# mlcolab/Pathfinder.jl

Hardware: AMD Instinct MI355X
Metric: ELBO draws/sec (multipathfinder hot path: fit + ELBO + pool + PSIS + resample) (higher is better)
Workload: dtype f64

## Files before the change

### pathfinder.jl_amd/csrc/elbo_qf_kernel.hip

```cpp
#include <type_traits>
#include <stdio.h>
#include <stdlib.h>
#include "pfmi_common.h"
#include "elbo_args.h"
#ifndef QF_PROF
#define QF_PROF 0
#endif

#ifndef QF_WAVES
#define QF_WAVES 8
#endif
#define QF_THREADS (QF_WAVES * 64)
#ifndef QF_NG
#define QF_NG 2
#endif
#ifndef QF_ABLATE
#define QF_ABLATE 0
#endif
#ifndef QF_NG2_MAXKC
#define QF_NG2_MAXKC 20
#endif
#ifndef QF_PRIO_FAIR
#define QF_PRIO_FAIR 8
#endif
#ifndef QF_PRIO_YOUNG
#define QF_PRIO_YOUNG 0
#endif
#ifndef QF_SETPRIO
#define QF_SETPRIO 0
#endif
#define QF_MIN_FRONT 1024
static_assert(QF_MIN_FRONT >= 2 * PF_ICDF_BFE_FRONT, "the look-up's front guard");
template <int KC> struct qf_chb { static constexpr int v = (KC > 20) ? 8 : 16; };

#pragma clang fp contract(off)

typedef double qf_d4 __attribute__((ext_vector_type(4)));
__device__ __forceinline__ qf_d4 qf_mfma16(double a, double b, qf_d4 c) { return __builtin_amdgcn_mfma_f64_16x16x4f64(a, b, c, 0, 0, 0); }
__device__ __forceinline__ double qf_mfma4(double a, double b, double c) { return __builtin_amdgcn_mfma_f64_4x4x4f64(a, b, c, 0, 0, 0); }

__host__ __device__ constexpr int qf_nconst(int KC, int RPAD) { return 4 + KC + KC * KC + RPAD + RPAD * KC + KC; }

template <int TGT>
__device__ __forceinline__ void qf_row_ac(const ElboArgs &A, const double *mu, int i, double &a, double &c) {
    if (TGT == 1) { a = A.t_a[i]; c = mu[i] - A.t_mean[i]; }
    else if (TGT == 2) { a = (i >= 1) ? 1.0 : 0.0; c = mu[i]; }
    else { a = 0.0; c = 0.0; }
}

template <int KC>
__device__ __forceinline__ int qf_vh_pos(int lrow, int col) {
    const int bl = lrow >> 4, rr = lrow & 15, q = rr >> 2, r = rr & 3, T = col >> 2, i = col & 3;
    return (((bl * 4 + r) * (KC / 4) + T) << 4) + q * 4 + i;
}

struct QfKernArgs { ElboArgs A; int ch_blocks, nchunks, groups_per_wg, ngroups, n_whole, n_tail, ndep; double *cshare; unsigned *cflag; unsigned epoch; };
#ifndef QF_SHARE_SPINS
#define QF_SHARE_SPINS 2000000
#endif
template <int KC, int TGT, int RPAD, int NG>
__global__ __launch_bounds__(QF_THREADS) void pf_elbo_qf_kernel(ElboArgs A, int ch_blocks, int nchunks, int groups_per_wg, int ngroups, int n_whole,
                                                                  int n_tail, int ndep, double *, unsigned *, unsigned) {
    extern __shared__ __attribute__((aligned(16))) double lds[];
#if QF_PROF
    const long long qf_t0 = wall_clock64();
    long long qf_tb = 0, qf_te = 0, qf_tp = 0, qf_last = 0;
#endif
    constexpr int NT = KC / 4, TR = RPAD / 4, NC = qf_nconst(KC, RPAD);
    constexpr int QF_CHB = qf_chb<KC>::v;
    constexpr bool FOLD = !(NG == 2 && KC >= 16);
    constexpr int PRE = (QF_CHB * 16 * KC + QF_THREADS - 1) / QF_THREADS;
    const int tid = threadIdx.x, wv = tid >> 6, lane = tid & 63, q = lane >> 4, c = lane & 15, l3 = lane & 3;
    const int d = A.d, nblk = (d + 15) >> 4;
    int slot = blockIdx.y, role = 0;
    int g_begin = blockIdx.x * groups_per_wg, g_cap = groups_per_wg;
    if (n_tail > 0 && slot >= n_whole) {
        constexpr int SL = QF_WAVES * NG, NPG_ = (TGT != 0) ? (KC + 1 + 15) / 16 : 0;
        int tail_f;
        if (slot < n_whole + n_tail) { role = 1; tail_f = slot - n_whole; g_begin = 0; g_cap = SL - NPG_; }
        else {
            const int t = slot - n_whole - n_tail;
            role = 2; tail_f = t / ndep;
            g_begin = (SL - NPG_) + (t - tail_f * ndep) * SL; g_cap = SL;
        }
        slot = n_whole + tail_f;
    }
    const int p = A.points[slot];
    const size_t blkidx = A.by_point ? (size_t)p : (size_t)slot;
    double *out_lp = A.logp + blkidx * A.log_stride, *out_lq = A.logq + blkidx * A.log_stride;
    constexpr int NPG = (TGT != 0) ? (KC + 1 + 15) / 16 : 0;
    const int npg = (role == 2) ? 0 : NPG;
    const int g_end = (g_begin + g_cap < ngroups) ? g_begin + g_cap : ngroups;
    const int nlb = (npg + (g_end - g_begin) + QF_WAVES * NG - 1) / (QF_WAVES * NG);
    if (A.status[p] != PFMI_FIT_OK) {
        for (int64_t n = (int64_t)g_begin * 16 + tid; n < (int64_t)g_end * 16 && n < A.N; n += QF_THREADS) {
            out_lp[n] = NAN; out_lq[n] = NAN;
        }
        return;
    }
    const int vh_sz = ch_blocks * 16 * KC, rs_sz = ch_blocks * 48;
    const int buf_stride = (nchunks > 1) ? vh_sz + rs_sz : 0;
    const int stage_sz = (nchunks > 1 ? 2 : 1) * (vh_sz + rs_sz);
    const int fix_off = stage_sz > QF_MIN_FRONT ? stage_sz : QF_MIN_FRONT;
    double *t_s = lds + fix_off;
    double *cn_s = t_s + KC * KC;
    double *g_s = cn_s + NC;
    double2 *icdf = reinterpret_cast<double2 *>(g_s + RPAD * RPAD + ((KC * KC + NC + RPAD * RPAD) & 1));

    const double *Vh = A.vh + (size_t)p * d * KC, *mu = A.mu + (size_t)p * d, *sqa = A.sqrt_alpha + (size_t)p * d;
    auto stage_direct = [&](int ck, int buf) {
        const int row0 = ck * ch_blocks * 16;
        double *vs = lds + buf * buf_stride, *rs = vs + vh_sz;
        const int npair = ch_blocks * 8 * KC;
        const int lim = (d - row0) * KC;
        const double2 *src = reinterpret_cast<const double2 *>(Vh + (size_t)row0 * KC);
        constexpr int U = 6;
        for (int j0 = tid; j0 < npair; j0 += QF_THREADS * U) {
            double2 v[U];
#pragma unroll
            for (int u = 0; u < U; ++u) {
                const int j = j0 + u * QF_THREADS, jc = (2 * j + 1 < lim) ? j : (lim >> 1) - 1;
                v[u] = src[jc];
            }
#pragma unroll
            for (int u = 0; u < U; ++u) {
                const int j = j0 + u * QF_THREADS, idx = 2 * j;
                if (j < npair) {
                    const int lrow = idx / KC, col = idx - lrow * KC;
                    const double2 val = (idx < lim) ? v[u] : make_double2(0.0, 0.0);
                    *reinterpret_cast<double2 *>(vs + qf_vh_pos<KC>(lrow, col)) = val;
                }
            }
        }
        for (int l0 = tid; l0 < ch_blocks * 16; l0 += QF_THREADS * 2) {
            double a[2], cc[2], s[2];
#pragma unroll
            for (int u = 0; u < 2; ++u) {
                const int lrow = l0 + u * QF_THREADS, row = row0 + lrow, rc = row < d ? row : d - 1;
                qf_row_ac<TGT>(A, mu, rc, a[u], cc[u]);
                s[u] = sqa[rc];
            }
#pragma unroll
            for (int u = 0; u < 2; ++u) {
                const int lrow = l0 + u * QF_THREADS, row = row0 + lrow;
                if (lrow < ch_blocks * 16) {
                    const bool in = row < d;
                    double *o = rs + (lrow >> 4) * 48 + (lrow & 15);
                    o[0] = in ? a[u] * s[u] * s[u] : 0.0; o[16] = in ? 2.0 * a[u] * cc[u] * s[u] : 0.0; o[32] = in ? s[u] : 0.0;
                }
            }
        }
    };
    {
        const double *T = A.tmat + (size_t)p * KC * KC;
        for (int i = tid; i < KC * KC; i += QF_THREADS) t_s[i] = T[i];
        for (int i = tid; i < NC; i += QF_THREADS) cn_s[i] = 0.0;
        if (RPAD > 0) for (int i = tid; i < RPAD * RPAD; i += QF_THREADS) g_s[i] = A.t_g[i];
        pf_icdf_load(icdf);
        stage_direct(0, 0);
    }
    const int rho = 4 * (c & 3) + (c >> 2);
    constexpr bool HREG = !(NG == 2 && KC >= 16);
    const double *Vc = A.vchol + (size_t)p * KC * KC;
    auto head_op = [&](const int which, const int r) -> double {
        const int b = 4 * q + r;
        if (which == 0) { double v = (rho == b) ? 1.0 : 0.0; if (rho < KC && b < KC) v = Vc[b * KC + rho]; return v; }
        const int i1 = 16 + rho, b1 = 16 + b;
        if (which == 1) return (i1 < KC) ? Vc[b * KC + i1] : 0.0;
        double v1 = (i1 == b1) ? 1.0 : 0.0;
        if (i1 < KC && b1 < KC) v1 = Vc[b1 * KC + i1];
        return v1;
    };
    double a_h00[HREG ? 4 : 1], a_h10[HREG ? 4 : 1], a_h11[HREG ? 4 : 1];
    if (HREG) {
#pragma unroll
        for (int r = 0; r < 4; ++r) {
            a_h00[HREG ? r : 0] = head_op(0, r);
            a_h10[HREG ? r : 0] = (KC > 16) ? head_op(1, r) : 0.0;
            a_h11[HREG ? r : 0] = (KC > 16) ? head_op(2, r) : 0.0;
        }
    }
    auto hop = [&](const int which, const int r) -> double {
        if (HREG) return which == 0 ? a_h00[HREG ? r : 0] : (which == 1 ? a_h10[HREG ? r : 0] : a_h11[HREG ? r : 0]);
        return head_op(which, r);
    };
    const uint64_t seed = A.seeds[slot];
    const uint32_t k0 = (uint32_t)seed, k1 = (uint32_t)(seed >> 32);
    const double logdet = A.logdet[p];
    __syncthreads();
#if QF_PROF
    qf_tp = wall_clock64() - qf_t0; qf_last = wall_clock64();
#endif
#if QF_PRIO_YOUNG
    if (wv >= 4) __builtin_amdgcn_s_setprio(1);
#endif
    if (TGT == 2) {
        if (tid == 0) { cn_s[1] = mu[0]; cn_s[2] = sqa[0]; }
        if (tid < KC) cn_s[4 + KC + KC * KC + RPAD + RPAD * KC + tid] = Vh[tid];
    }

    int cur = 0;
    for (int lb = 0; lb < nlb; ++lb) {
        bool pseudo[NG], active[NG];
        int sl[NG];
        int64_t nl[NG];
        uint32_t n[NG];
        double accw[NG][NT], acc3[NG][NT], acc4[NG][TR > 0 ? TR : 1];
        double usq[NG], q12[NG], z00[NG], u0[NG][4];
        bool any_active = false, any_pseudo = false, any_real = false;
#pragma unroll
        for (int g = 0; g < NG; ++g) {
            sl[g] = (lb * QF_WAVES + wv) * NG + g;
            pseudo[g] = sl[g] < npg;
            const int grp = g_begin + sl[g] - npg;
            active[g] = pseudo[g] || grp < g_end;
            nl[g] = (int64_t)grp * 16 + c;
            n[g] = (uint32_t)(A.n0 + nl[g]);
            any_active |= active[g]; any_pseudo |= pseudo[g]; any_real |= active[g] && !pseudo[g];
#pragma unroll
            for (int T = 0; T < NT; ++T) { accw[g][T] = 0.0; acc3[g][T] = 0.0; }
#pragma unroll
            for (int T = 0; T < (TR > 0 ? TR : 1); ++T) acc4[g][T] = 0.0;
            usq[g] = 0.0; q12[g] = 0.0; z00[g] = 0.0;
#pragma unroll
            for (int r = 0; r < 4; ++r) u0[g][r] = 0.0;
        }
        struct Pend { uint32_t x[4]; double dp[4]; double2 c01[4], c23[4]; };
        const uint32_t icdf_adj = pf_icdf_adj_bfe<PF_ICDF_NB_LDS>(icdf);
        auto gen_issue = [&](const int g, const int blk, Pend &P) {
#if QF_ABLATE == 1
#pragma unroll
            for (int r = 0; r < 4; ++r) { P.x[r] = 0x40000000u | (n[g] + blk); P.dp[r] = 1e-3 * (blk + r); P.c01[r] = make_double2(0.1, 0.2); P.c23[r] = make_double2(0.3, 0.4); }
#elif QF_ABLATE == 2
            pf_philox_normals(n[g], (uint32_t)(blk * 4 + q), 0u, 0u, k0, k1, P.x);
#pragma unroll
            for (int r = 0; r < 4; ++r) { P.dp[r] = (double)P.x[r] * 0x1p-32; P.c01[r] = make_double2(0.1, 0.2); P.c23[r] = make_double2(0.3, 0.4); }
#else
            pf_philox_normals(n[g], (uint32_t)(blk * 4 + q), 0u, 0u, k0, k1, P.x);
#pragma unroll
            for (int r = 0; r < 4; ++r) pf_icdf_issue_bfe<PF_ICDF_NB_LDS>(P.x[r], icdf_adj, P.dp[r], P.c01[r], P.c23[r]);
#endif
        };
        for (int ck = 0; ck < nchunks; ++ck) {
            double pre[PRE], pr_s = 0.0, pr_a = 0.0, pr_c = 0.0;
            const int nck = (ck + 1 < nchunks) ? ck + 1 : 0;
            const bool do_pre = (nchunks > 1) && (ck + 1 < nchunks || lb + 1 < nlb);
            if (do_pre) {
                const int row0 = nck * QF_CHB * 16;
                int tid_p = tid;
                asm volatile("" : "+v"(tid_p));
#pragma unroll
                for (int e = 0; e < PRE; ++e) {
                    const int idx = tid_p + e * QF_THREADS;
                    const int lrow = idx / KC, row = row0 + lrow;
                    pre[e] = (idx < QF_CHB * 16 * KC && row < d) ? Vh[(size_t)row0 * KC + idx] : 0.0;
                }
                if (tid_p < QF_CHB * 16) {
                    const int row = row0 + tid_p;
                    if (row < d) { qf_row_ac<TGT>(A, mu, row, pr_a, pr_c); pr_s = sqa[row]; }
                }
            }
            if (any_active) {
                const double *vs = lds + cur * buf_stride, *rs = vs + vh_sz;
                const int blk0 = ck * ch_blocks;
                const int nb = (nblk - blk0 < ch_blocks) ? nblk - blk0 : ch_blocks;
                struct Ops { double av[4][NT]; double wd[4][TR > 0 ? TR : 1]; double rs[12]; };
                auto load_ops = [&](const int bl, Ops &o) {
                    const double *rp = rs + bl * 48 + 4 * q;
                    const double *ap = vs + ((bl * 4) * NT << 4) + q * 4 + l3;
#pragma unroll
                    for (int r = 0; r < 4; ++r) {
#pragma unroll
                        for (int T = 0; T < NT; ++T) o.av[r][T] = ap[(r * NT + T) << 4];
                        o.rs[r] = rp[r]; o.rs[4 + r] = rp[16 + r]; o.rs[8 + r] = rp[32 + r];
                    }
                    if (TGT == 1 && RPAD > 0) {
                        const double *wp = A.t_wd16 + ((size_t)(blk0 + bl) * 16 + 4 * q) * 16 + l3;
#pragma unroll
                        for (int r = 0; r < 4; ++r)
#pragma unroll
                            for (int T = 0; T < TR; ++T) o.wd[r][T] = wp[r * 16 + 4 * T];
                    }
                };
                auto contract = [&](const int g, const double (&z)[4], const Ops &o, const bool with_w) {
#if QF_SETPRIO
                    __builtin_amdgcn_s_setprio(QF_SETPRIO);
#endif
                    double bp[4], bs[4];
#pragma unroll
                    for (int r = 0; r < 4; ++r) {
                        bp[r] = 0.0; bs[r] = 0.0;
                        if (TGT != 0) bp[r] = (with_w && FOLD) ? fma(o.rs[r], z[r], o.rs[4 + r]) : o.rs[r] * z[r];
                        if (TGT == 1 && RPAD > 0) bs[r] = o.rs[8 + r] * z[r];
                    }
                    __builtin_amdgcn_sched_barrier(0);
#pragma unroll
                    for (int r = 0; r < 4; ++r) {
                        if (TGT != 0) q12[g] = fma((with_w && FOLD) ? bp[r] : bp[r] + o.rs[4 + r], z[r], q12[g]);
#pragma unroll
                        for (int T = 0; T < NT; ++T) {
                            if (with_w) accw[g][T] = qf_mfma4(o.av[r][T], z[r], accw[g][T]);
                            if (TGT != 0) acc3[g][T] = qf_mfma4(o.av[r][T], bp[r], acc3[g][T]);
                        }
                        if (TGT == 1 && RPAD > 0) {
#pragma unroll
                            for (int T = 0; T < TR; ++T) acc4[g][T] = qf_mfma4(o.wd[r][T], bs[r], acc4[g][T]);
                        }
                    }
#if QF_SETPRIO
                    __builtin_amdgcn_s_setprio(0);
#endif
                };
                auto normals = [&](const int g, const int blk, double (&z)[4]) {
                    uint32_t x[4];
                    pf_philox_normals(n[g], (uint32_t)(blk * 4 + q), 0u, 0u, k0, k1, x);
                    pf_icdf4(x, n[g], (uint32_t)(blk * 4 + q), 0u, k0, k1, icdf, z);
                    if (blk == nblk - 1) {
#pragma unroll
                        for (int r = 0; r < 4; ++r) z[r] = (blk * 16 + 4 * q + r < d) ? z[r] : 0.0;
                    }
#pragma unroll
                    for (int r = 0; r < 4; ++r) usq[g] = fma(z[r], z[r], usq[g]);
                    if (blk == 0) {
                        qf_d4 h = {0.0, 0.0, 0.0, 0.0};
#pragma unroll
                        for (int r = 0; r < 4; ++r) { u0[g][r] = z[r]; h = qf_mfma16(hop(0, r), z[r], h); }
#pragma unroll
                        for (int r = 0; r < 4; ++r) z[r] = h[r];
                        z00[g] = z[0];
                    } else if (KC > 16 && blk == 1) {
                        qf_d4 h = {0.0, 0.0, 0.0, 0.0};
#pragma unroll
                        for (int r = 0; r < 4; ++r) h = qf_mfma16(hop(1, r), u0[g][r], h);
#pragma unroll
                        for (int r = 0; r < 4; ++r) h = qf_mfma16(hop(2, r), z[r], h);
#pragma unroll
                        for (int r = 0; r < 4; ++r) z[r] = h[r];
                    }
                };
                auto finish = [&](const int g, const int blk, const Pend &P, double (&z)[4], auto special_tag) {
                    constexpr bool SPECIAL = decltype(special_tag)::value;
#pragma unroll
                    for (int r = 0; r < 4; ++r) z[r] = pf_icdf_finish(P.x[r], P.dp[r], P.c01[r], P.c23[r]);
                    if (__builtin_expect(__any(pf_icdf_miss4(P.x)), 0))
                        pf_icdf4_fix(P.x, n[g], (uint32_t)(blk * 4 + q), 0u, k0, k1, z);
                    if (SPECIAL) {
                        if (blk == nblk - 1) {
#pragma unroll
                            for (int r = 0; r < 4; ++r) z[r] = (blk * 16 + 4 * q + r < d) ? z[r] : 0.0;
                        }
#pragma unroll
                        for (int r = 0; r < 4; ++r) usq[g] = fma(z[r], z[r], usq[g]);
                        if (blk == 0) {
                            qf_d4 h = {0.0, 0.0, 0.0, 0.0};
#pragma unroll
                            for (int r = 0; r < 4; ++r) { u0[g][r] = z[r]; h = qf_mfma16(hop(0, r), z[r], h); }
#pragma unroll
                            for (int r = 0; r < 4; ++r) z[r] = h[r];
                            z00[g] = z[0];
                        } else if (KC > 16 && blk == 1) {
                            qf_d4 h = {0.0, 0.0, 0.0, 0.0};
#pragma unroll
                            for (int r = 0; r < 4; ++r) h = qf_mfma16(hop(1, r), u0[g][r], h);
#pragma unroll
                            for (int r = 0; r < 4; ++r) h = qf_mfma16(hop(2, r), z[r], h);
#pragma unroll
                            for (int r = 0; r < 4; ++r) z[r] = h[r];
                        }
                    } else {
#pragma unroll
                        for (int r = 0; r < 4; ++r) usq[g] = fma(z[r], z[r], usq[g]);
                    }
                };
                auto pseudo_cols = [&](const int g, const int blk, const int bl, double (&z)[4]) {
                    const int j = 16 * sl[g] + c;
#pragma unroll
                    for (int r = 0; r < 4; ++r) {
                        const int row = blk * 16 + 4 * q + r;
                        double v = 0.0;
                        if (j < KC) v = vs[qf_vh_pos<KC>(bl * 16 + 4 * q + r, j)];
                        else if (j == KC && row < d) {
                            double aa, cc;
                            qf_row_ac<TGT>(A, mu, row, aa, cc);
                            v = cc / sqa[row];
                        }
                        z[r] = v;
                    }
                };
                if (any_pseudo) {
                    for (int bl = 0; bl < nb; ++bl) {
                        Ops oa;
                        load_ops(bl, oa);
#pragma unroll
                        for (int g = 0; g < NG; ++g) {
                            if (!active[g]) continue;
                            double z[4];
                            if (pseudo[g]) { pseudo_cols(g, blk0 + bl, bl, z); contract(g, z, oa, false); }
                            else { normals(g, blk0 + bl, z); contract(g, z, oa, true); }
                        }
                    }
                } else {
                    auto block_body_seq = [&](const int bl, auto special_tag) {
                        const int blk = blk0 + bl;
                        double z[NG][4];
#pragma unroll
                        for (int g = 0; g < NG; ++g) {
                            Pend pp;
                            gen_issue(g, blk, pp);
                            finish(g, blk, pp, z[g], special_tag);
                        }
                        const double *rp = rs + bl * 48 + 4 * q;
                        const double *ap = vs + ((bl * 4) * NT << 4) + q * 4 + l3;
#pragma unroll
                        for (int r = 0; r < 4; ++r) {
                            double av[NT];
#pragma unroll
                            for (int T = 0; T < NT; ++T) av[T] = ap[(r * NT + T) << 4];
                            const double r0 = rp[r], r1 = rp[16 + r];
#pragma unroll
                            for (int g = 0; g < NG; ++g) {
                                const double zr = z[g][r];
                                double bp = 0.0;
                                if (TGT != 0) {
                                    bp = r0 * zr;
                                    q12[g] = fma(bp + r1, zr, q12[g]);
                                }
#pragma unroll
                                for (int T = 0; T < NT; ++T) {
                                    accw[g][T] = qf_mfma4(av[T], zr, accw[g][T]);
                                    if (TGT != 0) acc3[g][T] = qf_mfma4(av[T], bp, acc3[g][T]);
                                }
                            }
                            if (TGT == 1 && RPAD > 0) {
                                const double *wp = A.t_wd16 + ((size_t)(blk0 + bl) * 16 + 4 * q + r) * 16 + l3;
                                double wd[TR > 0 ? TR : 1];
#pragma unroll
                                for (int T = 0; T < TR; ++T) wd[T] = wp[4 * T];
                                const double r2 = rp[32 + r];
#pragma unroll
                                for (int g = 0; g < NG; ++g) {
                                    const double bs = r2 * z[g][r];
#pragma unroll
                                    for (int T = 0; T < TR; ++T) acc4[g][T] = qf_mfma4(wd[T], bs, acc4[g][T]);
                                }
                            }
                        }
                    };
                    auto block_body = [&](const int bl, auto special_tag) {
                        if constexpr (NG == 2 && KC >= 16) { block_body_seq(bl, special_tag); return; }
                        const int blk = blk0 + bl;
                        Ops oa;
                        load_ops(bl, oa);
                        __builtin_amdgcn_sched_barrier(0);
                        Pend pp[NG];
                        double z[NG][4];
#pragma unroll
                        for (int g = 0; g < NG; ++g) gen_issue(g, blk, pp[g]);
#pragma unroll
                        for (int g = 0; g < NG; ++g) {
                            finish(g, blk, pp[g], z[g], special_tag);
#if QF_ABLATE == 3
                            q12[g] += z[g][0] + z[g][1] + z[g][2] + z[g][3] + oa.av[0][0] + oa.rs[0];
#else
                            contract(g, z[g], oa, true);
#endif
                        }
                    };
                    __builtin_amdgcn_s_waitcnt(0xC07F);
                    auto prio_turn = [&](const int blk) {
#if QF_PRIO_FAIR
                        if ((blk & (QF_PRIO_FAIR - 1)) == 0) {
                            if (((blk / QF_PRIO_FAIR) ^ (wv >> 2) ^ lb) & 1) __builtin_amdgcn_s_setprio(1); else __builtin_amdgcn_s_setprio(0);
                        }
#endif
                    };
                    if constexpr (NG == 2 && KC >= 16) {
                        for (int bl = 0; bl < nb; ++bl) {
                            const int blk = blk0 + bl;
                            prio_turn(blk);
                            if (__builtin_expect((blk == 0) | (blk == nblk - 1) | (KC > 16 && blk == 1), 0)) block_body(bl, std::true_type{});
                            else block_body(bl, std::false_type{});
                        }
                    } else {
                        constexpr int LEAD = (KC > 16) ? 2 : 1;
                        const int s_lo = (LEAD - blk0 <= 0) ? 0 : (LEAD - blk0 < nb ? LEAD - blk0 : nb);
                        const int s_hi = (blk0 + nb == nblk) ? (nb - 1 > s_lo ? nb - 1 : s_lo) : nb;
#pragma unroll
                        for (int bl = 0; bl < LEAD; ++bl)
                            if (bl < s_lo) { prio_turn(blk0 + bl); block_body(bl, std::true_type{}); }
                        for (int bl = s_lo; bl < s_hi; ++bl) { prio_turn(blk0 + bl); block_body(bl, std::false_type{}); }
                        if (s_hi < nb) { prio_turn(blk0 + s_hi); block_body(s_hi, std::true_type{}); }
                    }
                }
            }
            if (nchunks > 1) {
                if (do_pre) {
                    double *vs = lds + (cur ^ 1) * buf_stride, *rs = vs + vh_sz;
                    int tid_e = tid;
                    asm volatile("" : "+v"(tid_e));
#pragma unroll
                    for (int e = 0; e < PRE; ++e) {
                        const int idx = tid_e + e * QF_THREADS;
                        if (idx < QF_CHB * 16 * KC) { const int lrow = idx / KC; vs[qf_vh_pos<KC>(lrow, idx - lrow * KC)] = pre[e]; }
                    }
                    if (tid_e < QF_CHB * 16) {
                        double *o = rs + (tid_e >> 4) * 48 + (tid_e & 15);
                        o[0] = pr_a * pr_s * pr_s; o[16] = 2.0 * pr_a * pr_c * pr_s; o[32] = pr_s;
                    }
                }
                __syncthreads();
                cur ^= 1;
            }
        }
#if QF_PROF
        { const long long t_ = wall_clock64(); qf_tb += t_ - qf_last; qf_last = t_; }
#endif
        if (NPG > 0 && lb == 0) {
            int lane_p = lane;
            asm volatile("" : "+v"(lane_p));
            const int qp = lane_p >> 4, cp = lane_p & 15;
#pragma unroll
            for (int g = 0; g < NG; ++g) {
                if (!pseudo[g]) continue;
                const int j = 16 * sl[g] + cp;
                double *vv = cn_s + 4, *Mm = cn_s + 4 + KC, *t0 = Mm + KC * KC, *Nn = t0 + RPAD;
                const double q4 = pf_sum_q(q12[g]);
#pragma unroll
                for (int T = 0; T < NT; ++T) {
                    const int a = 4 * T + qp;
                    if (j < KC) Mm[a * KC + j] = acc3[g][T];
                    else if (j == KC) vv[a] = acc3[g][T];
                }
#pragma unroll
                for (int T = 0; T < TR; ++T) {
                    const int jr = 4 * T + qp;
                    if (j < KC) Nn[jr * KC + j] = acc4[g][T];
                    else if (j == KC) t0[jr] = acc4[g][T];
                }
                if (j == KC && qp == 0) cn_s[0] = q4 / 3.0;
            }
            double *cshare = nullptr; unsigned *cflag = nullptr; unsigned epoch = 0u; int tail_f = 0, n_tail_l = 0;
            if (role != 0) {
                const char *ka = (const char *)__builtin_amdgcn_kernarg_segment_ptr();
                asm volatile("" : "+s"(ka));
                cshare = *reinterpret_cast<double *const *>(ka + offsetof(QfKernArgs, cshare));
                cflag = *reinterpret_cast<unsigned *const *>(ka + offsetof(QfKernArgs, cflag));
                epoch = *reinterpret_cast<const unsigned *>(ka + offsetof(QfKernArgs, epoch));
                n_tail_l = *reinterpret_cast<const int *>(ka + offsetof(QfKernArgs, n_tail));
                const int n_whole_l = *reinterpret_cast<const int *>(ka + offsetof(QfKernArgs, n_whole));
                tail_f = slot - n_whole_l;
            }
            if (role == 2) {
                if (tid == 0) {
                    int spins = 0;
                    while (__hip_atomic_load(cflag + tail_f, __ATOMIC_ACQUIRE, __HIP_MEMORY_SCOPE_AGENT) != epoch && spins < QF_SHARE_SPINS) {
                        __builtin_amdgcn_s_sleep(32); ++spins;
                    }
                    if (spins >= QF_SHARE_SPINS) { cn_s[3] = NAN; atomicAdd(cflag + n_tail_l, 1u); }
                }
                __syncthreads();
                const bool lost = cn_s[3] != 0.0;
                const double *src = cshare + (size_t)tail_f * NC;
                double cv[(NC + QF_THREADS - 1) / QF_THREADS];
#pragma unroll
                for (int u = 0; u < (NC + QF_THREADS - 1) / QF_THREADS; ++u) {
                    const int i = tid + u * QF_THREADS;
                    cv[u] = __hip_atomic_load(src + (i < NC ? i : NC - 1), __ATOMIC_RELAXED, __HIP_MEMORY_SCOPE_AGENT);
                }
                __syncthreads();
#pragma unroll
                for (int u = 0; u < (NC + QF_THREADS - 1) / QF_THREADS; ++u) {
                    const int i = tid + u * QF_THREADS;
                    if (i < NC) cn_s[i] = lost ? NAN : cv[u];
                }
            }
            __syncthreads();
            if (role == 1) {
                double *dst = cshare + (size_t)tail_f * NC;
                for (int i = tid; i < NC; i += QF_THREADS) __hip_atomic_store(dst + i, cn_s[i], __ATOMIC_RELAXED, __HIP_MEMORY_SCOPE_AGENT);
                __threadfence();
                __syncthreads();
                if (tid == 0) __hip_atomic_store(cflag + tail_f, epoch, __ATOMIC_RELEASE, __HIP_MEMORY_SCOPE_AGENT);
            }
        }
        if (!any_real) continue;
        int lane_e = lane;
        asm volatile("" : "+v"(lane_e));
        const int qe = lane_e >> 4, ce = lane_e & 15;
#pragma unroll
        for (int g = 0; g < NG; ++g) {
            if (!active[g] || pseudo[g]) continue;
            double us = usq[g];
            us = pf_sum_q(us);
            double lp = NAN;
            if (TGT != 0) {
                double qs = q12[g];
                qs = pf_sum_q(qs);
                auto matvec = [&](const double *Mat, const int ld, const int nrows, auto nx_tag, auto ny_tag, auto lower_tag,
                                  const double (&x)[decltype(nx_tag)::value], double (&y)[decltype(ny_tag)::value]) {
                    constexpr int NX = decltype(nx_tag)::value, NY = decltype(ny_tag)::value;
                    constexpr bool LOWER = decltype(lower_tag)::value;
#pragma unroll
                    for (int rt = 0; rt < (NY + 3) / 4; ++rt) {
                        qf_d4 acc = {0.0, 0.0, 0.0, 0.0};
                        const int row = 16 * rt + ce;
#pragma unroll
                        for (int st = 0; st < NX; ++st) {
                            const int col = 4 * st + qe;
                            const bool ok = row < nrows && (!LOWER || col <= row);
                            const double av = ok ? Mat[row * ld + col] : 0.0;
                            acc = qf_mfma16(av, x[st], acc);
                        }
#pragma unroll
                        for (int r = 0; r < 4; ++r) if (4 * rt + r < NY) y[4 * rt + r] = acc[r];
                    }
                };
                const double *vv = cn_s + 4, *Mm = cn_s + 4 + KC, *t0 = Mm + KC * KC, *Nn = t0 + RPAD, *vh0 = Nn + RPAD * KC;
                double tvd[NT], mt[NT];
                matvec(t_s, KC, KC, std::integral_constant<int, NT>{}, std::integral_constant<int, NT>{}, std::false_type{}, accw[g], tvd);
                matvec(Mm, KC, KC, std::integral_constant<int, NT>{}, std::integral_constant<int, NT>{}, std::false_type{}, tvd, mt);
                double qa = 0.0;
#pragma unroll
                for (int T = 0; T < NT; ++T)
                    qa = fma(tvd[T], mt[T] - 2.0 * (FOLD ? acc3[g][T] - vv[4 * T + qe] : vv[4 * T + qe] + acc3[g][T]), qa);
                qa = pf_sum_q(qa);
                const double q1 = cn_s[0] + qs + qa;
                if (TGT == 1) {
                    double corr = 0.0;
                    if (RPAD > 0) {
                        constexpr int TRr = TR > 0 ? TR : 1;
                        double nt[TRr], tt[TRr], gg[TRr];
                        matvec(Nn, KC, RPAD, std::integral_constant<int, NT>{}, std::integral_constant<int, TRr>{}, std::false_type{}, tvd, nt);
#pragma unroll
                        for (int T = 0; T < TR; ++T) tt[T] = t0[4 * T + qe] + acc4[g][T] - nt[T];
                        matvec(g_s, RPAD, RPAD, std::integral_constant<int, TRr>{}, std::integral_constant<int, TRr>{}, std::true_type{}, tt, gg);
#pragma unroll
                        for (int T = 0; T < TR; ++T) corr = fma(gg[T], gg[T], corr);
                        corr = pf_sum_q(corr);
                    }
                    lp = A.t_offset - 0.5 * (q1 - corr);
                } else {
                    const double zh = __shfl(z00[g], ce, 64);
                    double pr = 0.0;
#pragma unroll
                    for (int T = 0; T < NT; ++T) pr = fma(vh0[4 * T + qe], tvd[T], pr);
                    pr = pf_sum_q(pr);
                    const double ta = cn_s[1] + cn_s[2] * (zh - pr), t3 = ta / 3.0;
                    lp = (t3 * t3 + (double)(d - 1) * ta + q1 * exp(-ta)) / -2.0;
                }
            }
            if (qe == 0 && nl[g] < A.N) {
                out_lq[nl[g]] = ((double)d * PF_LOG2PI + logdet + us) / -2.0;
                out_lp[nl[g]] = lp;
            }
        }
#if QF_PROF
        { const long long t_ = wall_clock64(); qf_te += t_ - qf_last; qf_last = t_; }
#endif
    }
#if QF_PROF
    if (g_begin == 0 && (slot & 1023) == 3 && lane == 0)
        printf("QF_PROF fit %d wave %d (10 ns ticks): prologue %lld blocks %lld epilogue+publish %lld total %lld batches %d\n", slot, wv, qf_tp, qf_tb,
               qf_te, (long long)(wall_clock64() - qf_t0), nlb);
#endif
}

static size_t qf_lds_bytes(int ch_blocks, int nchunks, int kc, int rpad) {
    const size_t per = (size_t)ch_blocks * 16 * kc + (size_t)ch_blocks * 48;
    size_t stage = per * (nchunks > 1 ? 2 : 1);
    if (stage < QF_MIN_FRONT) stage = QF_MIN_FRONT;
    return sizeof(double) * (stage + (size_t)kc * kc + qf_nconst(kc, rpad) + (size_t)rpad * rpad + 1 + 4 * PF_ICDF_LDS_ENTRIES + 2 * PF_ICDF_BFE_BEHIND);
}

static void qf_note_plan(pfmi_ctx *c, int kc, int tgt, int rpad, int ng, bool streamed, const char *cut) {
    char nm[64];
    snprintf(nm, sizeof nm, "qf:%d,%d,%d,%d:%s:%s", kc, tgt, rpad, ng, streamed ? "stream" : "res", cut);
    ++c->qf_plans[nm];
}

template <int KC, int TGT, int RPAD, int NG>
static int32_t launch_qf_ng(pfmi_ctx *c, const ElboArgs &a, int64_t nfits) {
    const int nblk = (a.d + 15) / 16;
    int ch_blocks = nblk, nchunks = 1;
    constexpr int QF_CHB = qf_chb<KC>::v;
    if (qf_lds_bytes(nblk, 1, KC, RPAD) > 156 * 1024) { ch_blocks = QF_CHB; nchunks = (nblk + QF_CHB - 1) / QF_CHB; }
    const size_t lds_bytes = qf_lds_bytes(ch_blocks, nchunks, KC, RPAD);
    PF_CHECK(lds_bytes <= 160 * 1024, PFMI_ERR_UNSUPPORTED, "qf kernel LDS %zu too large", lds_bytes);
    auto kern = pf_elbo_qf_kernel<KC, TGT, RPAD, NG>;
    PF_TRY(pf_raise_lds_limit(c, reinterpret_cast<const void *>(kern), 160 * 1024));
    const int ngroups = (int)((a.N + 15) / 16);
    constexpr int NPG = (TGT != 0) ? (KC + 1 + 15) / 16 : 0;
    int split = 1;
    while (!c->qf_seg_mode && (int64_t)split * nfits < 1024 && (ngroups + NPG) / (split * 2) >= QF_WAVES * NG) split *= 2;
    int gpw = (ngroups + split - 1) / split;
    if (split > 1) gpw = ((gpw + NPG + QF_WAVES * NG - 1) / (QF_WAVES * NG)) * (QF_WAVES * NG) - NPG;
    if (gpw < 1) gpw = 1;
    const int gx = (ngroups + gpw - 1) / gpw;
    auto launch = [&](int64_t f0, int64_t nf, int gpw_, int gx_) {
        for (int64_t s0 = f0; s0 < f0 + nf; s0 += 32768) {
            const int64_t ns = (f0 + nf - s0 < 32768) ? (f0 + nf - s0) : 32768;
            ElboArgs b = a;
            b.points = a.points + s0; b.seeds = a.seeds + s0;
            if (!a.by_point) { b.logp += s0 * a.log_stride; b.logq += s0 * a.log_stride; }
            hipLaunchKernelGGL(kern, dim3((unsigned)gx_, (unsigned)ns), dim3(QF_THREADS), lds_bytes, c->stream, b, ch_blocks, nchunks, gpw_,
                               ngroups, 0, 0, 0, (double *)nullptr, (unsigned *)nullptr, 0u);
        }
    };
    int64_t tail = 0;
    int gpw_t = gpw, gx_t = gx, ndep = 0;
    const char *no_tail = pf_debug_get("PFMI_QF_NO_TAIL");
    const char *two = pf_debug_get("PFMI_QF_TWO_LAUNCHES");
    const bool two_launches = (two && two[0] == '1') || c->qf_no_share;
    if (split == 1 && TGT != 0 && !(no_tail && no_tail[0] == '1') && !c->qf_seg_mode) {
        int ncu = 0;
        PF_HIP(hipDeviceGetAttribute(&ncu, hipDeviceAttributeMultiprocessorCount, c->device));
        if (c->ncu_eff > 0 && c->ncu_eff < ncu) ncu = c->ncu_eff;
        const int slots = QF_WAVES * NG, nb_full = (ngroups + NPG + slots - 1) / slots;
        const int64_t rem = ncu > 0 ? nfits % ncu : 0;
        gpw_t = slots - NPG;
        gx_t = gpw_t > 0 ? (ngroups + gpw_t - 1) / gpw_t : 0;
        ndep = (ngroups > gpw_t) ? (ngroups - gpw_t + slots - 1) / slots : 0;
        const bool share_ok = !two_launches && gpw_t > 0 && (nfits - rem) + rem * (1 + ndep) <= 65535;
        const int pieces = share_ok ? 1 + ndep : gx_t;
        if (rem > 0 && nfits > ncu && gpw_t > 0 && nb_full > 1 && (rem * pieces + ncu - 1) / ncu < nb_full) tail = rem;
        if (tail > 0 && share_ok) {
            constexpr int NC = qf_nconst(KC, RPAD);
            const size_t cbytes = (size_t)tail * NC * sizeof(double), fbytes = ((size_t)tail + 1) * sizeof(unsigned);
            DevBuf &share = c->qf_share_s[c->qf_slot];
            uint32_t &epoch = c->qf_epoch_s[c->qf_slot];
            if (share.cap < cbytes + fbytes || epoch == 0xFFFFFFFFu) {
                PF_CHECK(!c->stream_pending, PFMI_ERR_STATE, "scan: the hand-over buffer of a streaming call must be allocated before its first launch");
                PF_TRY(share.ensure(cbytes + fbytes + (64 << 10)));
                PF_HIP(hipMemsetAsync(share.p, 0, share.cap, c->stream));
                epoch = 0;
            }
            unsigned *cflag = reinterpret_cast<unsigned *>(share.as<char>() + share.cap) - (tail + 1);
            hipLaunchKernelGGL(kern, dim3(1, (unsigned)((nfits - tail) + tail * (1 + ndep))), dim3(QF_THREADS), lds_bytes, c->stream, a, ch_blocks,
                               nchunks, gpw, ngroups, (int)(nfits - tail), (int)tail, ndep, share.as<double>(), cflag, ++epoch);
            qf_note_plan(c, KC, TGT, RPAD, NG, nchunks > 1, "tail-share");
            return PFMI_OK;
        }
    }
    if (nfits - tail > 0) launch(0, nfits - tail, gpw, gx);
    if (tail > 0) launch(nfits - tail, tail, gpw_t, gx_t);
    qf_note_plan(c, KC, TGT, RPAD, NG, nchunks > 1, tail > 0 ? "tail-two" : (split > 1 ? "split" : "whole"));
    return PFMI_OK;
}

template <int KC, int TGT, int RPAD>
static int32_t launch_qf(pfmi_ctx *c, const ElboArgs &a, int64_t nfits) {
    if constexpr (KC <= QF_NG2_MAXKC && QF_NG == 2) {
        if (a.N >= 768 && (KC <= 12 || nfits >= 128)) return launch_qf_ng<KC, TGT, RPAD, 2>(c, a, nfits);
    }
    return launch_qf_ng<KC, TGT, RPAD, 1>(c, a, nfits);
}

template <int KC>
static int32_t launch_qf_t(pfmi_ctx *c, const ElboArgs &a, int64_t nfits, int tgt, int rpad) {
    if (tgt == 0) return launch_qf<KC, 0, 0>(c, a, nfits);
    if (tgt == 2) return launch_qf<KC, 2, 0>(c, a, nfits);
    if (rpad == 0) return launch_qf<KC, 1, 0>(c, a, nfits);
    if (rpad == 8) return launch_qf<KC, 1, 8>(c, a, nfits);
    return launch_qf<KC, 1, 16>(c, a, nfits);
}

int32_t pf_launch_elbo_qf(pfmi_ctx *c, const ElboArgs &a, int64_t nfits, int tgt, int rpad, bool *handled) {
    *handled = false;
    if (a.u != nullptr || a.x != nullptr) return PFMI_OK;
    int32_t rc = PFMI_OK;
    *handled = pf_dispatch_kpad<4, 8, 12, 16, 20, 32>(c->kpad, [&](auto KP) { rc = launch_qf_t<KP()>(c, a, nfits, tgt, rpad); });
    return rc;
}
```

Before: 507.2 million.

## Precompute M·T and N·T products per fit and batch epilogue MFMAs across groups

The per-sample epilogue previously ran a chain of matvecs (T·w, then M·(T·w), then N·(T·w), then G·…) with fresh LDS operand loads for every group. The change precomputes P1 = M·T and P2 = N·T once per fit into shared constants. This turns the chained matvecs into independent MFMAs on accw, whose operands are loaded once and reused across the NG groups. The cross-lane reductions are also batched across groups, and the T/G staging loads are hoisted into registers so they overlap with other prologue work. The cost is a larger constant block (more LDS and more shared-publish traffic) and a slight change in floating-point rounding order.

```diff
diff --git a/pathfinder.jl_amd/csrc/elbo_qf_kernel.hip b/pathfinder.jl_amd/csrc/elbo_qf_kernel.hip
--- a/pathfinder.jl_amd/csrc/elbo_qf_kernel.hip
+++ b/pathfinder.jl_amd/csrc/elbo_qf_kernel.hip
@@ -39,7 +39,7 @@
 __device__ __forceinline__ qf_d4 qf_mfma16(double a, double b, qf_d4 c) { return __builtin_amdgcn_mfma_f64_16x16x4f64(a, b, c, 0, 0, 0); }
 __device__ __forceinline__ double qf_mfma4(double a, double b, double c) { return __builtin_amdgcn_mfma_f64_4x4x4f64(a, b, c, 0, 0, 0); }
 
-__host__ __device__ constexpr int qf_nconst(int KC, int RPAD) { return 4 + KC + KC * KC + RPAD + RPAD * KC + KC; }
+__host__ __device__ constexpr int qf_nconst(int KC, int RPAD) { return 4 + KC + KC * KC + RPAD + RPAD * KC + KC + KC * KC + RPAD * KC; }
 
 template <int TGT>
 __device__ __forceinline__ void qf_row_ac(const ElboArgs &A, const double *mu, int i, double &a, double &c) {
@@ -64,7 +64,7 @@
     extern __shared__ __attribute__((aligned(16))) double lds[];
 #if QF_PROF
     const long long qf_t0 = wall_clock64();
-    long long qf_tb = 0, qf_te = 0, qf_tp = 0, qf_last = 0;
+    long long qf_tb = 0, qf_te = 0, qf_tp = 0, qf_tc = 0, qf_last = 0;
 #endif
     constexpr int NT = KC / 4, TR = RPAD / 4, NC = qf_nconst(KC, RPAD);
     constexpr int QF_CHB = qf_chb<KC>::v;
@@ -151,14 +151,6 @@
             }
         }
     };
-    {
-        const double *T = A.tmat + (size_t)p * KC * KC;
-        for (int i = tid; i < KC * KC; i += QF_THREADS) t_s[i] = T[i];
-        for (int i = tid; i < NC; i += QF_THREADS) cn_s[i] = 0.0;
-        if (RPAD > 0) for (int i = tid; i < RPAD * RPAD; i += QF_THREADS) g_s[i] = A.t_g[i];
-        pf_icdf_load(icdf);
-        stage_direct(0, 0);
-    }
     const int rho = 4 * (c & 3) + (c >> 2);
     constexpr bool HREG = !(NG == 2 && KC >= 16);
     const double *Vc = A.vchol + (size_t)p * KC * KC;
@@ -187,6 +179,21 @@
     const uint64_t seed = A.seeds[slot];
     const uint32_t k0 = (uint32_t)seed, k1 = (uint32_t)(seed >> 32);
     const double logdet = A.logdet[p];
+    {
+        static_assert(RPAD * RPAD <= QF_THREADS, "G is staged with one load per thread");
+        constexpr int TQ = (KC * KC + QF_THREADS - 1) / QF_THREADS;
+        const double *T = A.tmat + (size_t)p * KC * KC;
+        double tq[TQ], gq = 0.0;
+#pragma unroll
+        for (int u = 0; u < TQ; ++u) { const int i = tid + u * QF_THREADS; tq[u] = T[i < KC * KC ? i : KC * KC - 1]; }
+        if (RPAD > 0) gq = A.t_g[tid < RPAD * RPAD ? tid : 0];
+        for (int i = tid; i < NC; i += QF_THREADS) cn_s[i] = 0.0;
+        pf_icdf_load(icdf);
+        stage_direct(0, 0);
+#pragma unroll
+        for (int u = 0; u < TQ; ++u) { const int i = tid + u * QF_THREADS; if (i < KC * KC) t_s[i] = tq[u]; }
+        if (RPAD > 0 && tid < RPAD * RPAD) g_s[tid] = gq;
+    }
     __syncthreads();
 #if QF_PROF
     qf_tp = wall_clock64() - qf_t0; qf_last = wall_clock64();
@@ -198,6 +205,42 @@
         if (tid == 0) { cn_s[1] = mu[0]; cn_s[2] = sqa[0]; }
         if (tid < KC) cn_s[4 + KC + KC * KC + RPAD + RPAD * KC + tid] = Vh[tid];
     }
+
+    auto matvec_ops = [&](const double *Mat, const int ld, const int nrows, const int qq, const int cc, auto lower_tag, auto &a) {
+        using Arr = std::remove_reference_t<decltype(a)>;
+        constexpr int NR = std::extent<Arr, 0>::value, NX = std::extent<Arr, 1>::value;
+        constexpr bool LOWER = decltype(lower_tag)::value;
+#pragma unroll
+        for (int rt = 0; rt < NR; ++rt) {
+            const int row = 16 * rt + cc;
+#pragma unroll
+            for (int st = 0; st < NX; ++st) {
+                const int col = 4 * st + qq;
+                const bool ok = row < nrows && (!LOWER || col <= row);
+                a[rt][st] = ok ? Mat[row * ld + col] : 0.0;
+            }
+        }
+    };
+    auto matvec = [&](const double *Mat, const int ld, const int nrows, const int qq, const int cc, auto nx_tag, auto ny_tag, auto lower_tag,
+                      const double (&x)[decltype(nx_tag)::value], double (&y)[decltype(ny_tag)::value]) {
+        constexpr int NX = decltype(nx_tag)::value, NY = decltype(ny_tag)::value;
+        double a[(NY + 3) / 4][NX];
+        matvec_ops(Mat, ld, nrows, qq, cc, lower_tag, a);
+#pragma unroll
+        for (int rt = 0; rt < (NY + 3) / 4; ++rt) {
+            qf_d4 acc = {0.0, 0.0, 0.0, 0.0};
+#pragma unroll
+            for (int st = 0; st < NX; ++st) acc = qf_mfma16(a[rt][st], x[st], acc);
+#pragma unroll
+            for (int r = 0; r < 4; ++r) if (4 * rt + r < NY) y[4 * rt + r] = acc[r];
+        }
+    };
+    auto qf_sum_q_all = [](double (&v)[NG]) {
+#pragma unroll
+        for (int g = 0; g < NG; ++g) v[g] = pf_add_xor16(v[g]);
+#pragma unroll
+        for (int g = 0; g < NG; ++g) v[g] = pf_add_xor32(v[g]);
+    };
 
     int cur = 0;
     for (int lb = 0; lb < nlb; ++lb) {
@@ -519,11 +562,11 @@
             int lane_p = lane;
             asm volatile("" : "+v"(lane_p));
             const int qp = lane_p >> 4, cp = lane_p & 15;
+            double *vv = cn_s + 4, *Mm = cn_s + 4 + KC, *t0 = Mm + KC * KC, *Nn = t0 + RPAD, *P1 = Nn + RPAD * KC + KC, *P2 = P1 + KC * KC;
 #pragma unroll
             for (int g = 0; g < NG; ++g) {
                 if (!pseudo[g]) continue;
                 const int j = 16 * sl[g] + cp;
-                double *vv = cn_s + 4, *Mm = cn_s + 4 + KC, *t0 = Mm + KC * KC, *Nn = t0 + RPAD;
                 const double q4 = pf_sum_q(q12[g]);
 #pragma unroll
                 for (int T = 0; T < NT; ++T) {
@@ -539,43 +582,64 @@
                 }
                 if (j == KC && qp == 0) cn_s[0] = q4 / 3.0;
             }
-            double *cshare = nullptr; unsigned *cflag = nullptr; unsigned epoch = 0u; int tail_f = 0, n_tail_l = 0;
+            double *cshare = nullptr; unsigned *cflag = nullptr; unsigned epoch = 0u; int tail_f = 0;
             if (role != 0) {
                 const char *ka = (const char *)__builtin_amdgcn_kernarg_segment_ptr();
                 asm volatile("" : "+s"(ka));
                 cshare = *reinterpret_cast<double *const *>(ka + offsetof(QfKernArgs, cshare));
                 cflag = *reinterpret_cast<unsigned *const *>(ka + offsetof(QfKernArgs, cflag));
                 epoch = *reinterpret_cast<const unsigned *>(ka + offsetof(QfKernArgs, epoch));
-                n_tail_l = *reinterpret_cast<const int *>(ka + offsetof(QfKernArgs, n_tail));
+                const int n_tail_l = *reinterpret_cast<const int *>(ka + offsetof(QfKernArgs, n_tail));
                 const int n_whole_l = *reinterpret_cast<const int *>(ka + offsetof(QfKernArgs, n_whole));
                 tail_f = slot - n_whole_l;
-            }
-            if (role == 2) {
-                if (tid == 0) {
-                    int spins = 0;
-                    while (__hip_atomic_load(cflag + tail_f, __ATOMIC_ACQUIRE, __HIP_MEMORY_SCOPE_AGENT) != epoch && spins < QF_SHARE_SPINS) {
-                        __builtin_amdgcn_s_sleep(32); ++spins;
-                    }
-                    if (spins >= QF_SHARE_SPINS) { cn_s[3] = NAN; atomicAdd(cflag + n_tail_l, 1u); }
-                }
+                if (role == 2) {
+                    if (tid == 0) {
+                        int spins = 0;
+                        while (__hip_atomic_load(cflag + tail_f, __ATOMIC_ACQUIRE, __HIP_MEMORY_SCOPE_AGENT) != epoch && spins < QF_SHARE_SPINS) {
+                            __builtin_amdgcn_s_sleep(32); ++spins;
+                        }
+                        if (spins >= QF_SHARE_SPINS) { cn_s[3] = NAN; atomicAdd(cflag + n_tail_l, 1u); }
+                    }
+                    __syncthreads();
+                    const bool lost = cn_s[3] != 0.0;
+                    const double *src = cshare + (size_t)tail_f * NC;
+                    double cv[(NC + QF_THREADS - 1) / QF_THREADS];
+                    int tid_c = tid;
+                    asm volatile("" : "+v"(tid_c));
+#pragma unroll
+                    for (int u = 0; u < (NC + QF_THREADS - 1) / QF_THREADS; ++u) {
+                        const int i = tid_c + u * QF_THREADS;
+                        cv[u] = __hip_atomic_load(src + (i < NC ? i : NC - 1), __ATOMIC_RELAXED, __HIP_MEMORY_SCOPE_AGENT);
+                    }
+                    __syncthreads();
+#pragma unroll
+                    for (int u = 0; u < (NC + QF_THREADS - 1) / QF_THREADS; ++u) {
+                        const int i = tid_c + u * QF_THREADS;
+                        if (i < NC) cn_s[i] = lost ? NAN : cv[u];
+                    }
+                }
+            }
+            __syncthreads();
+            if (role != 2) {
+#pragma unroll
+                for (int ct = 0; ct < (KC + 15) / 16; ++ct) {
+                    const int j = 16 * ct + cp;
+                    double tc[NT], y1[NT], y2[TR > 0 ? TR : 1];
+#pragma unroll
+                    for (int st = 0; st < NT; ++st) tc[st] = (j < KC) ? t_s[(4 * st + qp) * KC + j] : 0.0;
+                    matvec(Mm, KC, KC, qp, cp, std::integral_constant<int, NT>{}, std::integral_constant<int, NT>{}, std::false_type{}, tc, y1);
+                    if (TGT == 1 && RPAD > 0)
+                        matvec(Nn, KC, RPAD, qp, cp, std::integral_constant<int, NT>{}, std::integral_constant<int, (TR > 0 ? TR : 1)>{}, std::false_type{}, tc, y2);
+#pragma unroll
+                    for (int T = 0; T < NT; ++T) if (j < KC) P1[(4 * T + qp) * KC + j] = y1[T];
+                    if (TGT == 1 && RPAD > 0) {
+#pragma unroll
+                        for (int T = 0; T < TR; ++T) if (j < KC) P2[(4 * T + qp) * KC + j] = y2[T];
+                    }
+                }
+            }
+            if (role == 1) {
                 __syncthreads();
-                const bool lost = cn_s[3] != 0.0;
-                const double *src = cshare + (size_t)tail_f * NC;
-                double cv[(NC + QF_THREADS - 1) / QF_THREADS];
-#pragma unroll
-                for (int u = 0; u < (NC + QF_THREADS - 1) / QF_THREADS; ++u) {
-                    const int i = tid + u * QF_THREADS;
-                    cv[u] = __hip_atomic_load(src + (i < NC ? i : NC - 1), __ATOMIC_RELAXED, __HIP_MEMORY_SCOPE_AGENT);
-                }
-                __syncthreads();
-#pragma unroll
-                for (int u = 0; u < (NC + QF_THREADS - 1) / QF_THREADS; ++u) {
-                    const int i = tid + u * QF_THREADS;
-                    if (i < NC) cn_s[i] = lost ? NAN : cv[u];
-                }
-            }
-            __syncthreads();
-            if (role == 1) {
                 double *dst = cshare + (size_t)tail_f * NC;
                 for (int i = tid; i < NC; i += QF_THREADS) __hip_atomic_store(dst + i, cn_s[i], __ATOMIC_RELAXED, __HIP_MEMORY_SCOPE_AGENT);
                 __threadfence();
@@ -583,75 +647,100 @@
                 if (tid == 0) __hip_atomic_store(cflag + tail_f, epoch, __ATOMIC_RELEASE, __HIP_MEMORY_SCOPE_AGENT);
             }
         }
+#if QF_PROF
+        { const long long t_ = wall_clock64(); qf_tc += t_ - qf_last; qf_last = t_; }
+#endif
         if (!any_real) continue;
         int lane_e = lane;
         asm volatile("" : "+v"(lane_e));
         const int qe = lane_e >> 4, ce = lane_e & 15;
-#pragma unroll
-        for (int g = 0; g < NG; ++g) {
-            if (!active[g] || pseudo[g]) continue;
-            double us = usq[g];
-            us = pf_sum_q(us);
-            double lp = NAN;
-            if (TGT != 0) {
-                double qs = q12[g];
-                qs = pf_sum_q(qs);
-                auto matvec = [&](const double *Mat, const int ld, const int nrows, auto nx_tag, auto ny_tag, auto lower_tag,
-                                  const double (&x)[decltype(nx_tag)::value], double (&y)[decltype(ny_tag)::value]) {
-                    constexpr int NX = decltype(nx_tag)::value, NY = decltype(ny_tag)::value;
-                    constexpr bool LOWER = decltype(lower_tag)::value;
-#pragma unroll
-                    for (int rt = 0; rt < (NY + 3) / 4; ++rt) {
-                        qf_d4 acc = {0.0, 0.0, 0.0, 0.0};
-                        const int row = 16 * rt + ce;
-#pragma unroll
-                        for (int st = 0; st < NX; ++st) {
-                            const int col = 4 * st + qe;
-                            const bool ok = row < nrows && (!LOWER || col <= row);
-                            const double av = ok ? Mat[row * ld + col] : 0.0;
-                            acc = qf_mfma16(av, x[st], acc);
-                        }
-#pragma unroll
-                        for (int r = 0; r < 4; ++r) if (4 * rt + r < NY) y[4 * rt + r] = acc[r];
-                    }
-                };
-                const double *vv = cn_s + 4, *Mm = cn_s + 4 + KC, *t0 = Mm + KC * KC, *Nn = t0 + RPAD, *vh0 = Nn + RPAD * KC;
-                double tvd[NT], mt[NT];
-                matvec(t_s, KC, KC, std::integral_constant<int, NT>{}, std::integral_constant<int, NT>{}, std::false_type{}, accw[g], tvd);
-                matvec(Mm, KC, KC, std::integral_constant<int, NT>{}, std::integral_constant<int, NT>{}, std::false_type{}, tvd, mt);
-                double qa = 0.0;
+        double us[NG], lp[NG];
+#pragma unroll
+        for (int g = 0; g < NG; ++g) { us[g] = usq[g]; if (TGT == 0) lp[g] = NAN; }
+        if (TGT != 0) {
+            constexpr int TRr = TR > 0 ? TR : 1, NRT = (NT + 3) / 4, NRR = (TRr + 3) / 4;
+            constexpr bool LR = (TGT == 1 && RPAD > 0);
+            const double *vv = cn_s + 4, *t0 = vv + KC + KC * KC, *vh0 = t0 + RPAD + RPAD * KC, *P1 = vh0 + KC, *P2 = P1 + KC * KC;
+            double aT[NRT][NT], a1[NRT][NT], a2[NRR][NT], aG[NRR][TRr];
+            matvec_ops(t_s, KC, KC, qe, ce, std::false_type{}, aT);
+            matvec_ops(P1, KC, KC, qe, ce, std::false_type{}, a1);
+            if (LR) { matvec_ops(P2, KC, RPAD, qe, ce, std::false_type{}, a2); matvec_ops(g_s, RPAD, RPAD, qe, ce, std::true_type{}, aG); }
+            qf_d4 cT[NG][NRT], c1[NG][NRT], c2[NG][NRR], cG[NG][NRR];
+#pragma unroll
+            for (int g = 0; g < NG; ++g) {
+#pragma unroll
+                for (int rt = 0; rt < NRT; ++rt) { cT[g][rt] = qf_d4{0.0, 0.0, 0.0, 0.0}; c1[g][rt] = qf_d4{0.0, 0.0, 0.0, 0.0}; }
+#pragma unroll
+                for (int rt = 0; rt < NRR; ++rt) { c2[g][rt] = qf_d4{0.0, 0.0, 0.0, 0.0}; cG[g][rt] = qf_d4{0.0, 0.0, 0.0, 0.0}; }
+            }
+#pragma unroll
+            for (int st = 0; st < NT; ++st) {
+#pragma unroll
+                for (int g = 0; g < NG; ++g) {
+#pragma unroll
+                    for (int rt = 0; rt < NRT; ++rt) {
+                        cT[g][rt] = qf_mfma16(aT[rt][st], accw[g][st], cT[g][rt]);
+                        c1[g][rt] = qf_mfma16(a1[rt][st], accw[g][st], c1[g][rt]);
+                    }
+                    if (LR) {
+#pragma unroll
+                        for (int rt = 0; rt < NRR; ++rt) c2[g][rt] = qf_mfma16(a2[rt][st], accw[g][st], c2[g][rt]);
+                    }
+                }
+            }
+            double tt[NG][TRr], qs[NG], qa[NG], corr[NG];
+            if (LR) {
+#pragma unroll
+                for (int g = 0; g < NG; ++g)
+#pragma unroll
+                    for (int T = 0; T < TR; ++T) tt[g][T] = t0[4 * T + qe] + acc4[g][T] - c2[g][T >> 2][T & 3];
+#pragma unroll
+                for (int st = 0; st < TR; ++st)
+#pragma unroll
+                    for (int g = 0; g < NG; ++g)
+#pragma unroll
+                        for (int rt = 0; rt < NRR; ++rt) cG[g][rt] = qf_mfma16(aG[rt][st], tt[g][st], cG[g][rt]);
+            }
+#pragma unroll
+            for (int g = 0; g < NG; ++g) {
+                qs[g] = q12[g]; qa[g] = 0.0; corr[g] = 0.0;
 #pragma unroll
                 for (int T = 0; T < NT; ++T)
-                    qa = fma(tvd[T], mt[T] - 2.0 * (FOLD ? acc3[g][T] - vv[4 * T + qe] : vv[4 * T + qe] + acc3[g][T]), qa);
-                qa = pf_sum_q(qa);
-                const double q1 = cn_s[0] + qs + qa;
+                    qa[g] = fma(cT[g][T >> 2][T & 3], c1[g][T >> 2][T & 3] - 2.0 * (FOLD ? acc3[g][T] - vv[4 * T + qe] : vv[4 * T + qe] + acc3[g][T]), qa[g]);
+            }
+            qf_sum_q_all(us); qf_sum_q_all(qs); qf_sum_q_all(qa);
+#pragma unroll
+            for (int g = 0; g < NG; ++g) {
+                const double q1 = cn_s[0] + qs[g] + qa[g];
                 if (TGT == 1) {
-                    double corr = 0.0;
-                    if (RPAD > 0) {
-                        constexpr int TRr = TR > 0 ? TR : 1;
-                        double nt[TRr], tt[TRr], gg[TRr];
-                        matvec(Nn, KC, RPAD, std::integral_constant<int, NT>{}, std::integral_constant<int, TRr>{}, std::false_type{}, tvd, nt);
-#pragma unroll
-                        for (int T = 0; T < TR; ++T) tt[T] = t0[4 * T + qe] + acc4[g][T] - nt[T];
-                        matvec(g_s, RPAD, RPAD, std::integral_constant<int, TRr>{}, std::integral_constant<int, TRr>{}, std::true_type{}, tt, gg);
-#pragma unroll
-                        for (int T = 0; T < TR; ++T) corr = fma(gg[T], gg[T], corr);
-                        corr = pf_sum_q(corr);
-                    }
-                    lp = A.t_offset - 0.5 * (q1 - corr);
+                    if (LR) {
+#pragma unroll
+                        for (int T = 0; T < TR; ++T) corr[g] = fma(cG[g][T >> 2][T & 3], cG[g][T >> 2][T & 3], corr[g]);
+                    }
+                    lp[g] = q1;
                 } else {
                     const double zh = __shfl(z00[g], ce, 64);
                     double pr = 0.0;
 #pragma unroll
-                    for (int T = 0; T < NT; ++T) pr = fma(vh0[4 * T + qe], tvd[T], pr);
+                    for (int T = 0; T < NT; ++T) pr = fma(vh0[4 * T + qe], cT[g][T >> 2][T & 3], pr);
                     pr = pf_sum_q(pr);
                     const double ta = cn_s[1] + cn_s[2] * (zh - pr), t3 = ta / 3.0;
-                    lp = (t3 * t3 + (double)(d - 1) * ta + q1 * exp(-ta)) / -2.0;
-                }
-            }
-            if (qe == 0 && nl[g] < A.N) {
-                out_lq[nl[g]] = ((double)d * PF_LOG2PI + logdet + us) / -2.0;
-                out_lp[nl[g]] = lp;
+                    lp[g] = (t3 * t3 + (double)(d - 1) * ta + q1 * exp(-ta)) / -2.0;
+                }
+            }
+            if (TGT == 1) {
+                if (LR) qf_sum_q_all(corr);
+#pragma unroll
+                for (int g = 0; g < NG; ++g) lp[g] = A.t_offset - 0.5 * (lp[g] - corr[g]);
+            }
+        } else {
+            qf_sum_q_all(us);
+        }
+#pragma unroll
+        for (int g = 0; g < NG; ++g) {
+            if (active[g] && !pseudo[g] && qe == 0 && nl[g] < A.N) {
+                out_lq[nl[g]] = ((double)d * PF_LOG2PI + logdet + us[g]) / -2.0;
+                out_lp[nl[g]] = lp[g];
             }
         }
 #if QF_PROF
@@ -659,9 +748,10 @@
 #endif
     }
 #if QF_PROF
-    if (g_begin == 0 && (slot & 1023) == 3 && lane == 0)
-        printf("QF_PROF fit %d wave %d (10 ns ticks): prologue %lld blocks %lld epilogue+publish %lld total %lld batches %d\n", slot, wv, qf_tp, qf_tb,
-               qf_te, (long long)(wall_clock64() - qf_t0), nlb);
+    const bool qf_show = role == 0 ? (g_begin == 0 && (slot & 1023) == 3) : (slot == n_whole && g_begin <= QF_WAVES * NG);
+    if (qf_show && lane == 0)
+        printf("QF_PROF fit %d role %d wave %d (10 ns ticks): prologue %lld blocks %lld publish %lld epilogue %lld total %lld batches %d\n", slot, role, wv,
+               qf_tp, qf_tb, qf_tc, qf_te, (long long)(wall_clock64() - qf_t0), nlb);
 #endif
 }
 
```

Result: no change. 509.8 million, median of 6 (+0.5%).
